# lixiaobai09/xgnn

Measured on AMD Instinct MI355X. Metric: sampled edges/s + feature-extract GB/s per epoch-step, higher is better.
Workload: dtype u32 ids / f32 rows (bit copy)

## Files before the change

### include/ggms.h

```cpp
#ifndef GGMS_H
#define GGMS_H

#include <stddef.h>
#include <stdint.h>

#ifdef __cplusplus
extern "C" {
#endif

typedef uint32_t ggms_id_t;
typedef void *ggms_stream_t;
typedef void *ggms_event_t;
#define GGMS_EMPTY_KEY 0xffffffffu

enum ggms_status {
  GGMS_OK = 0,
  GGMS_ERR_INVALID = -1,
  GGMS_ERR_HIP = -2,
  GGMS_ERR_NO_DEVICE = -3
};

enum ggms_dtype {
  GGMS_F32 = 0,
  GGMS_F64 = 1,
// ... 30 lines not shown
#define GGMS_DEBUG_GRID_CAP 3
#define GGMS_DEBUG_NUM_KNOBS 4
void ggms_debug_set_knob(int knob, long long value);
size_t ggms_dtype_bytes(int dtype);
size_t ggms_row_bytes(int dtype, size_t dim);

#define GGMS_MAX_PARTS 8
typedef struct {
  const ggms_id_t *indptr;
  const ggms_id_t *indices;
  const ggms_id_t *const *part_indptr;
  const ggms_id_t *const *part_indices;
  uint32_t num_part;
  uint32_t num_cache_node;
  uint32_t num_node;
  uint32_t _pad;
} ggms_graph_t;

#define GGMS_RNG_STATE_BYTES 24
int ggms_random_states_init(void *states, size_t num_states, uint64_t seed,
                            ggms_stream_t stream);
size_t ggms_random_states_count(int sample_type, const size_t *fanout,
                                size_t num_fanout, size_t batch_size,
                                size_t num_random_walk);

enum ggms_sample_type {
  GGMS_KHOP0 = 0,
  GGMS_KHOP1 = 1,
  GGMS_WEIGHTED_KHOP = 2,
  GGMS_RANDOM_WALK = 3,
  GGMS_WEIGHTED_KHOP_PREFIX = 4,
  GGMS_KHOP2 = 5,
// ... 439 lines not shown
```

### xgnn_amd/_lib.py

```python
import ctypes as C
import os

_HERE = os.path.dirname(os.path.abspath(__file__))
LIB_PATH = os.path.join(_HERE, "lib", "libggms_hip.so")
_LIB = None


class GgmsError(RuntimeError):
    pass


class Graph(C.Structure):
    _fields_ = [("indptr", C.c_void_p), ("indices", C.c_void_p),
                ("part_indptr", C.c_void_p), ("part_indices", C.c_void_p),
                ("num_part", C.c_uint32), ("num_cache_node", C.c_uint32),
                ("num_node", C.c_uint32), ("_pad", C.c_uint32)]


class SampleExtra(C.Structure):
    _fields_ = [("prob_table", C.c_void_p), ("alias_table", C.c_void_p), ("random_walk_length", C.c_size_t),
                ("random_walk_restart_prob", C.c_double), ("num_random_walk", C.c_size_t), ("data", C.c_void_p),
                ("rng_wait", C.c_void_p), ("rng_done", C.c_void_p), ("heavy_wait", C.c_void_p),
                ("seeds_distinct", C.c_uint32), ("labor_salt", C.c_uint32)]


class Temporal(C.Structure):
    _fields_ = [("edge_time", C.c_void_p), ("cut_table", C.c_void_p), ("stamp", C.c_uint32), ("pick", C.c_uint32)]


class Typed(C.Structure):
    _fields_ = [("edge_type", C.c_void_p), ("num_type", C.c_uint32), ("type_fanout", C.POINTER(C.c_uint32))]
# ... 56 lines not shown


_vp, _sz, _u64, _u32, _i = C.c_void_p, C.c_size_t, C.c_uint64, C.c_uint32, C.c_int
SYMBOLS = {
    "ggms_abi_version": (_i, []),
    "ggms_last_error": (C.c_char_p, []),
    "ggms_device_status": (_i, [C.POINTER(_u32), _i]),
    "ggms_debug_poison_next_scan": (None, []),
    "ggms_debug_set_scan_patience": (None, [C.c_uint32]),
    "ggms_debug_delay_next_scan": (None, [C.c_uint32]),
    "ggms_debug_set_scan_epoch": (C.c_uint32, [C.c_uint32]),
    "ggms_debug_set_knob": (None, [_i, C.c_longlong]),
    "ggms_fabric_probe": (_i, [_i, _vp, _sz, _sz, _u32, _vp, _vp]),
    "ggms_dtype_bytes": (_sz, [_i]),
    "ggms_row_bytes": (_sz, [_i, _sz]),
    "ggms_random_states_init": (_i, [_vp, _sz, _u64, _vp]),
    "ggms_random_states_count": (_sz, [_i, C.POINTER(_sz), _sz, _sz, _sz]),
    "ggms_sample_workspace_bytes": (_sz, [_i, _sz, _sz]),
    "ggms_sample_khop3": (_i, [C.POINTER(Graph), _vp, _sz, _sz, _vp, _vp, _vp, _vp, _sz, _vp, _sz, _vp]),
    "ggms_sample_khop0": (_i, [C.POINTER(Graph), _vp, _sz, _sz, _vp, _vp, _vp, _vp, _sz, _vp]),
    "ggms_sample_khop_labor": (_i, [C.POINTER(Graph), _vp, _sz, _sz, C.c_uint32, _vp, _vp, _vp, _vp, _sz, _vp]),
    "ggms_sample_khop_temporal": (_i, [C.POINTER(Graph), _vp, _vp, _vp, _sz, _sz, _i, C.c_uint32, _vp, _vp, _vp, _vp, _vp,
                                       _sz, _vp]),
    "ggms_sample_khop1": (_i, [C.POINTER(Graph), _vp, _sz, _sz, _vp, _vp, _vp, _vp, _sz, _vp, _sz, _vp]),
    "ggms_sample_khop2": (_i, [C.POINTER(Graph), _vp, _sz, _sz, _vp, _vp, _vp, _vp, _sz, _vp, _sz, _vp]),
    "ggms_sample_weighted_workspace_bytes": (_sz, [_sz, _sz]),
    "ggms_sample_weighted_khop": (_i, [C.POINTER(Graph), _vp, _vp, _vp, _sz, _sz, _vp, _vp, _vp, _vp, _sz, _vp, _sz,
                                       _vp]),
    "ggms_sample_weighted_khop_prefix": (_i, [C.POINTER(Graph), _vp, _vp, _sz, _sz, _vp, _vp, _vp, _vp, _sz, _vp, _sz,
                                              _vp]),
# ... 125 lines not shown
```

### xgnn_amd/csrc/engine/engine.cc

```cpp
#include "engine.h"
#include "team.h"
#include "../labor_hash.h"
#include "../row_formats.h"

#include <fcntl.h>
#include <pthread.h>
#include <sys/mman.h>
#include <signal.h>
#include <sys/stat.h>
#include <sys/wait.h>
#include <unistd.h>

#include <algorithm>
#include <atomic>
#include <chrono>
#include <condition_variable>
#include <cstdio>
#include <cstdlib>
#include <cstring>
#include <fstream>
#include <iostream>
#include <memory>
#include <mutex>
#include <random>
// ... 217 lines not shown
    const std::string v = kv["feat_store_dtype"];
    const auto name = kFeatDtypeNames.find(v);
    if (name == kFeatDtypeNames.end() || !ggms::quantiser_writes(name->second))
      fatal(__FILE__, __LINE__, "feat_store_dtype = " + v + ": unknown store type; the GPU quantiser writes F16, BF16, "
                                "F8E4M3, F8E5M2 or Q8ROW");
    cfg.feat_store_dtype = name->second;
    if (cfg.arch == kArch0)
      fatal(__FILE__, __LINE__, "arch0: feat_store_dtype needs a GPU: the table is encoded by a kernel, and the CPU engine "
                                "has no GPU; quantise the dataset offline (datagen.quantize_features)");
    if (cfg.arch == kArch5 || cfg.arch == kArch6)
      fatal(__FILE__, __LINE__, std::string(cfg.arch == kArch5 ? "arch5" : "arch6") + ": feat_store_dtype is not built: the "
                                "process that loads the dataset forks its workers and must not initialise the GPU before it "
                                "forks; quantise the dataset offline (datagen.quantize_features)");
    if (cfg.feat_store_dtype == GGMS_Q8ROW && cfg.feat_out_dtype < 0) fatal(__FILE__, __LINE__, kQ8RowNeedsOutDtype);
  }
  if (kv.count("task")) {
    const std::string v = kv["task"];
    if (v != "node_classification" && v != "link_prediction")
      fatal(__FILE__, __LINE__, "task = " + v + ": node_classification (the default) or link_prediction");
    cfg.link_prediction = v == "link_prediction";
  }
  if (cfg.link_prediction) {
    static const char *const arch_names[] = {"arch0", "arch1", "arch2", "arch3", "arch4", "arch5", "arch6", "arch7"};
    if (cfg.arch != kArch1)
      fatal(__FILE__, __LINE__, std::string(arch_names[cfg.arch]) + ": task = link_prediction is not built: edge seeds, "
                                "negative sampling and the pair ids run in arch1's sampling chain only");
    if (cfg.sample_type == GGMS_RANDOM_WALK)
      fatal(__FILE__, __LINE__, "task = link_prediction with _sample_type 3 (random_walk) is not built: the pair ids are "
                                "the k-hop batch's seed ids");
    if (kv.count("num_negative")) {
// ... 734 lines not shown
  void *d = nullptr;
  SAM_HIP(hipHostGetDevicePointer(&d, host, 0));
  return d;
}

void Engine::UploadGraph() {
  const uint32_t *indptr = (const uint32_t *)ds.indptr.ptr, *indices = (const uint32_t *)ds.indices.ptr;
  std::memset(&graph_, 0, sizeof(graph_));
  graph_.num_node = (uint32_t)ds.num_node;
  if (!cfg.use_dist_graph) {
    d_indptr_ = (uint32_t *)dev_upload(indptr, ds.indptr.bytes, stream_);
    d_indices_ = (uint32_t *)dev_upload(indices, ds.indices.bytes, stream_);
    graph_.indptr = d_indptr_;
    graph_.indices = d_indices_;
    SAM_HIP(hipStreamSynchronize(stream_));
    return;
  }
  const uint32_t P = (uint32_t)cfg.num_worker, p = (uint32_t)worker_id_;
  const uint32_t num_cache_edge = (uint32_t)(ds.num_edge * cfg.dist_graph_percentage);
  uint32_t num_cache_node = 0;
  while (num_cache_node < ds.num_node && indptr[num_cache_node] < num_cache_edge) ++num_cache_node;
  const size_t isz = num_cache_node / P + (p < num_cache_node % P ? 1 : 0) + 1;
  std::vector<uint32_t> pip(isz);
  size_t ecount = 0;
  for (uint32_t v = p; v < num_cache_node; v += P) ecount += indptr[v + 1] - indptr[v];
  std::vector<uint32_t> pix(std::max<size_t>(ecount, 1));
  uint32_t cnt = 0;
  for (uint32_t v = p; v < num_cache_node; v += P) {
    const uint32_t ne = indptr[v + 1] - indptr[v];
    pip[v / P] = cnt;
// ... 15 lines not shown
    for (uint32_t q = 0; q < P; ++q) {
      if (q == p) continue;
      part_indptr_[q] = OpenPeer(shared_->graph_indptr[q], q, shared_->indptr_words[q] * 4, "graph indptr shard");
      part_indices_[q] = OpenPeer(shared_->graph_indices[q], q, shared_->indices_words[q] * 4, "graph indices shard");
    }
    Barrier("graph shards opened");
  }
  part_indptr_[P] = dev_upload(ds.indptr.ptr, ds.indptr.bytes, stream_);
  SAM_HIP(hipStreamSynchronize(stream_));
  part_indices_[P] = (void *)map_host(ds.indices.ptr, ds.indices.bytes);
  SAM_CHECK(P <= GGMS_MAX_PARTS, "use_dist_graph: at most GGMS_MAX_PARTS topology shards");
  graph_.part_indptr = (const ggms_id_t *const *)part_indptr_.data();
  graph_.part_indices = (const ggms_id_t *const *)part_indices_.data();
  graph_.num_part = P;
  graph_.num_cache_node = num_cache_node;
}

void Engine::ComputeBounds() {
  const uint32_t L = (uint32_t)cfg.fanout.size();
  max_seeds_ = (size_t)(cfg.batch_size * 1.25) + 1;
  if (cfg.link_prediction) max_seeds_ = cfg.batch_size * (2 + cfg.num_negative);
  max_input_.resize(L);
  max_edges_.resize(L);
  SAM_GGMS(ggms_sample_batch_capacity(max_seeds_, cfg.fanout.data(), L, max_input_.data(), max_edges_.data(), &max_unique_));
  if (cfg.arch == kArch4)
    SAM_GGMS(ggms_sample_batch_prefetch_capacity(max_seeds_, cfg.fanout.data(), L, (const ggms_id_t *)ds.indptr.ptr,
                                                 ds.num_node, cfg.prefetch_max_edges, &max_prefetch_edges_, &max_unique_));
}

void Engine::SampleInit(int worker_id, const std::string &ctx) {
// ... 544 lines not shown
void Engine::Start() {
  if (Dedicated()) ExtractStart(0);
}

void Engine::Shutdown() {
  shutdown_ = true;
  bg_stop_ = true;
  pool_cv_.notify_all();
  if (bg_.joinable()) bg_.join();
  if (cfg.arch == kArch0) CpuShutdown();
  for (auto &P : pipes_)
    if (P.stream) (void)hipStreamSynchronize(P.stream);
  if (stream_) (void)hipStreamSynchronize(stream_);
  if (stream_extract_) (void)hipStreamSynchronize(stream_extract_);
  if (stream_extract2_) (void)hipStreamSynchronize(stream_extract2_);
}

Batch *Engine::AcquireSlot(bool background) {
  for (;;) {
    {
      std::lock_guard<std::mutex> lk(pool_mu_);
      for (auto &b : slots_)
        if (!b->in_use && b->refs.load() == 0) { b->in_use = true; return b.get(); }
    }
    if (bg_stop_) return nullptr;
    if (!background) return nullptr;
    std::this_thread::sleep_for(std::chrono::microseconds(20));
  }
}

// ... 505 lines not shown
```

### xgnn_amd/csrc/engine/engine.h

```cpp
#pragma once

#include <hip/hip_runtime.h>

#include <atomic>
#include <condition_variable>
#include <cstdint>
#include <deque>
#include <map>
#include <memory>
#include <mutex>
#include <string>
#include <thread>
#include <unordered_map>
#include <vector>

#include "../../../include/ggms.h"
#include "../../../include/samgraph.h"

namespace sam {

[[noreturn]] void fatal(const char *file, int line, const std::string &msg);
#define SAM_CHECK(cond, msg)                                   \
  do {                                                         \
    if (!(cond)) ::sam::fatal(__FILE__, __LINE__, std::string("Check failed: " #cond " ") + (msg)); \
// ... 35 lines not shown
  bool part_cache = false, gpu_extract = false;
  double replicate_percentage = 0.0;
  bool configured = false;
  bool has_seed = false;
  uint64_t seed = 0;
  uint64_t labor_seed = 0;
  bool direct_table = true;
  size_t lookahead = 2;
  size_t extract_streams = 2;
  size_t pipelines = 1;
  size_t presample_epoch = 0;
  bool dynamic_cache = false;
  size_t prefetch_max_edges = (size_t)1 << 26;
  int feat_out_dtype = -1;
  int feat_store_dtype = -1;
  bool link_prediction = false;
  uint32_t num_negative = 1;
  int negative_mode = GGMS_NEG_EXCLUDE;
  uint32_t exclude_seed_edges = 0;
  int feat_learnable = -1;
  float feat_lr = 0.0f, feat_eps = 1e-10f;
  bool edge_ids = false, edge_feat = false;
  int temporal_pick = GGMS_PICK_UNIFORM;
  bool Temporal() const { return sample_type == GGMS_KHOP_TEMPORAL; }
  std::vector<uint32_t> type_fanout;
  uint32_t num_edge_type = 0;
  bool Typed() const { return sample_type == GGMS_KHOP_TYPED; }
  bool SamplerEmitsEdgeIds() const { return Temporal() || Typed(); }
  bool induced = false;
  size_t induced_max_edges = 0;
// ... 151 lines not shown
  void *OpenPeer(const hipIpcMemHandle_t &handle, uint32_t peer, size_t bytes, const char *what);

 private:
  void LoadDataset();
  HostArray MapFile(const std::string &name, size_t bytes, bool to_shared_anon);
  void ShufflerInit();
  const uint32_t *SeedSet() const { return cfg.link_prediction ? ds.train_edges : (const uint32_t *)ds.train_set.ptr; }
  size_t SeedSetSize() const { return cfg.link_prediction ? ds.num_train_edge : ds.num_train; }
  uint64_t link_forced_ = 0;
  bool ShufflerNext(Batch *b, hipStream_t copy_stream);
  void Reshuffle();
  void DetectTopo();
  ggms_topology_t topo_{};
  bool topo_valid_ = false;
  void UploadGraph();
  void Presample();
  void QuantizeStore();
  void BuildCache();
  Batch *AcquireSlot(bool background);
  bool StagedHostTier() const { return cfg.arch == kArch6 && !cfg.gpu_extract && (cache_table_ != nullptr || !cfg.UseGPUCache()); }
  void StagedExtract(Batch *b, hipStream_t ss, hipStream_t xs);
  void HostGatherRows(char *rows, const uint32_t *ids, size_t first, size_t count);
  std::unique_ptr<class Team> host_team_;
  size_t staged_batches_ = 0;
  void SanityCheckBatch(const uint32_t *seeds, size_t n);
  std::vector<bool> sanity_seen_;
  uint32_t *node_access_dev_ = nullptr;
 public:
  void ReportNodeAccess();
 private:
// ... 25 lines not shown
  bool QueueWait(const uint64_t *word, uint64_t want, const char *what, bool stoppable);
  void PublishRanking();
  void WaitRankingReady();
  void Arch5TrainerInit(int worker_id, const std::string &ctx);
  void SendOne();
  bool Receive(Batch *b);
  void Unpack(Batch *b, hipStream_t xs);

  bool data_ready_ = false, sample_ready_ = false, train_ready_ = false, shutdown_ = false;
  int worker_id_ = 0, device_ = 0;
  int trainer_device_ = 0;
  hipStream_t stream_ = nullptr;
  hipStream_t stream_extract_ = nullptr;
  hipStream_t stream_extract2_ = nullptr;
  uint32_t *d_indptr_ = nullptr, *d_indices_ = nullptr;
  std::vector<void *> part_indptr_, part_indices_;
  ggms_graph_t graph_{};
  ggms_hashtable_t ht_{};
  ggms_sample_extra_t extra_{};
  void *d_prob_ = nullptr, *d_alias_ = nullptr;
  void *states_ = nullptr;
  size_t num_states_ = 0;
  void *ws_ = nullptr;
  size_t ws_bytes_ = 0;
  struct Pipe {
    hipStream_t stream = nullptr;
    ggms_hashtable_t ht{};
    void *ws = nullptr;
    hipEvent_t rng_done = nullptr;
    void *drop_ws = nullptr;
// ... 60 lines not shown
```

### xgnn_amd/csrc/ggms_device.h

```cpp
#pragma once
#include <cstdlib>

#include <hip/hip_runtime.h>
#include <stdint.h>

#include "../../include/ggms.h"

namespace ggms {

constexpr uint32_t kEmptyKey = GGMS_EMPTY_KEY;
constexpr int kWave = 64;
constexpr int kBlock = 256;
constexpr int kMaxGridBlocks = 2048;

void set_error(const char *fmt, ...);
#define GGMS_CHECK_ARG(cond)                                              \
  do {                                                                    \
    if (!(cond)) {                                                        \
      ::ggms::set_error("%s:%d: invalid argument: %s", __FILE__, __LINE__, #cond); \
      return GGMS_ERR_INVALID;                                            \
    }                                                                     \
  } while (0)
#define GGMS_HIP(call)                                                    \
  do {                                                                    \
// ... 56 lines not shown
  __device__ __forceinline__ T *pick(uint32_t k) const {
    T *r = p[0];
#pragma unroll 1
    for (uint32_t i = 1; i < N; ++i) r = (k == i) ? p[i] : r;
    return r;
  }
};

struct GraphView {
  const uint32_t *indptr;
  const uint32_t *indices;
  PtrSet<const uint32_t, kMaxParts + 1> pip, pix;
  Divisor part;
  uint32_t num_part;
  uint32_t num_cache_node;

  typedef uint32_t u32x2_a4 __attribute__((ext_vector_type(2), aligned(4)));
  static __device__ __forceinline__ void bounds(const uint32_t *ip, uint32_t v, uint32_t &b, uint32_t &e) {
    const u32x2_a4 be = *reinterpret_cast<const u32x2_a4 *>(ip + v);
    b = be.x;
    e = be.y;
  }
  __device__ __forceinline__ const uint32_t *neighbours(uint32_t v, uint32_t &len) const {
    if (num_part == 0) {
      uint32_t b, e;
      bounds(indptr, v, b, e);
      len = e - b;
      return indices + b;
    }
    uint32_t slot, real;
    part.divmod(v, real, slot);
    const bool cached = v < num_cache_node;
    slot = cached ? slot : kMaxParts;
    real = cached ? real : v;
    uint32_t b, e;
    bounds(pip.pick(slot), real, b, e);
    len = e - b;
    return pix.pick(slot) + b;
  }
};

bool host_readable_table(const void *table, const char *what);

inline bool view_of(const ggms_graph_t *g, GraphView &v) {
  v = GraphView{};
  v.indptr = g->indptr;
  v.indices = g->indices;
  v.num_part = g->num_part;
  v.num_cache_node = g->num_cache_node;
  v.part = divisor_of(g->num_part ? g->num_part : 1);
  if (g->num_part == 0) return true;
  if (g->num_part > kMaxParts || !g->part_indptr || !g->part_indices) {
    set_error("graph view: num_part %u (at most %u shards; part_indptr / part_indices are HOST arrays of num_part + 1 device pointers)",
              g->num_part, kMaxParts);
    return false;
  }
  if (!host_readable_table(g->part_indptr, "ggms_graph_t.part_indptr") ||
      !host_readable_table(g->part_indices, "ggms_graph_t.part_indices"))
    return false;
  for (uint32_t p = 0; p < g->num_part; ++p) {
    v.pip.p[p] = g->part_indptr[p];
    v.pix.p[p] = g->part_indices[p];
  }
  v.pip.p[kMaxParts] = g->part_indptr[g->num_part];
  v.pix.p[kMaxParts] = g->part_indices[g->num_part];
  return true;
// ... 134 lines not shown
```

### xgnn_amd/csrc/sample_khop.hip

```cpp
#include <algorithm>
#include <atomic>

#include "ggms_internal.h"

namespace ggms {

struct SeedCount {
  GraphView g;
  const uint32_t *input;
  uint32_t fanout;
  __device__ __forceinline__ uint32_t operator()(uint64_t i) const {
    uint32_t len;
    g.neighbours(input[i], len);
    return len < fanout ? len : fanout;
  }
};
struct StoreOffset {
  uint32_t *offset;
  __device__ __forceinline__ void operator()(uint64_t i, uint32_t, uint32_t excl) const { offset[i] = excl; }
};

template <int S>
__device__ __forceinline__ uint32_t row_shr(uint32_t v) {
  return (uint32_t)__builtin_amdgcn_update_dpp(0, (int)v, 0x110 + S, 0xf, 0xf, true);
}

struct Khop3TileHelp {
  static constexpr bool kCan = true;
  const GraphView &g;
  const uint32_t *input;
  uint64_t n;
  uint32_t fanout;
  __device__ __forceinline__ uint32_t operator()(uint64_t t) const {
    uint32_t acc = 0;
#pragma unroll
    for (uint32_t k = 0; k < 2; ++k) {
      const uint64_t i = 128 * t + 64 * k + (threadIdx.x & 63u);
      if (i < n) {
        uint32_t len;
        (void)g.neighbours(input[i], len);
        acc += len < fanout ? len : fanout;
      }
    }
    return wave_reduce_sum(acc);
  }
};

template <int GPW, bool INSERT, bool FIRST>
__global__ __launch_bounds__(128 * (4 / GPW), 6) void k_khop3_fused(GraphView g, const uint32_t *__restrict__ input,
                                                                 Count n_arg, uint32_t fanout, uint32_t fanout_magic,
                                                                 uint32_t *__restrict__ out_src,
                                                                 uint32_t *__restrict__ out_dst, SrcMode sm,
                                                                 uint32_t *__restrict__ states, uint32_t set_mask,
                                                                 uint32_t multi, FusedScan fs, DedupInsert di,
                                                                 FirstLayer fl) {
  constexpr uint32_t HASH_EMPTY = 0xffffffffu, NT = 128 * (4 / GPW), FLAG_A = 1, FLAG_P = 2;
  extern __shared__ uint32_t s_pos[];
  __shared__ uint32_t set_tab[8][128];
  __shared__ const uint32_t *s_ptr[128];
  __shared__ uint32_t s_len[128], s_rid[128], s_off[129];
  __shared__ uint64_t s_tile;
  __shared__ uint32_t s_prefix;
  const uint32_t lane = threadIdx.x & 63u;
  const bool active = GPW == 4 || lane < 16u * GPW;
  const uint64_t n = n_arg.get();
  if constexpr (FIRST) {
    if (blockIdx.x == 0) fl.pro.run(n, threadIdx.x, NT);
  }
  const uint32_t y = (threadIdx.x >> 6) * GPW + (lane >> 4), lig = lane & 15u;
  const uint32_t grp_shift = lane & ~15u;
  uint32_t *const tab = set_tab[active ? y : 0];
  const uint64_t num_tiles = (n + 127) / 128;
  const uint32_t my_s = y + 8u * lig;

  if (active)
    for (uint32_t s = lig; s <= set_mask; s += 16) tab[s] = HASH_EMPTY;
  bool dirty = false;

  const bool one_tile_each = gridDim.x >= num_tiles;
  for (uint32_t turn = 0;; ++turn) {
    if (one_tile_each) {
      if (turn != 0) break;
    } else {
      if (threadIdx.x == 0) s_tile = take_ticket(fs.tick);
      __syncthreads();
    }
    const uint64_t b = one_tile_each ? (uint64_t)blockIdx.x : s_tile;
    if (b >= num_tiles) break;
    uint32_t my_len = 0, my_magic = 0;
    unsigned long long seed_old = 0;
    if (active) {
      const uint64_t my_index = 128 * b + my_s;
      const uint32_t *ptr = nullptr;
      uint32_t rid = 0;
      if (my_index < n) {
        rid = input[my_index];
        if constexpr (FIRST) {
          fl.n2o[my_index] = rid;
          seed_old = atomicMin(di.w + rid, make_w1(di.version, 1u, (uint32_t)my_index));
        }
        ptr = g.neighbours(rid, my_len);
        if (my_len > fanout) my_magic = (uint32_t)(4294967296.0 / (double)my_len);
      }
      s_ptr[my_s] = ptr;
      s_len[my_s] = my_len;
      s_rid[my_s] = rid;
    }
    __syncthreads();
    if (threadIdx.x < kWave) {
      const uint32_t a = min(s_len[2 * lane], fanout), c = min(s_len[2 * lane + 1], fanout);
      const uint32_t incl = wave_inclusive_scan(a + c);
      s_off[2 * lane] = incl - (a + c);
      s_off[2 * lane + 1] = incl - c;
      if (lane == 63) {
        s_off[128] = incl;
        __hip_atomic_store(&fs.desc[b], scan_desc(fs.epoch, b == 0 ? FLAG_P : FLAG_A, incl), __ATOMIC_RELAXED,
// ... 100 lines not shown
        }
        if (lig == 0) st.store(states + 6 * stream);
      }
    }
    if constexpr (FIRST) {
      const uint64_t my_index = 128 * b + my_s;
      if (active && my_index < n) {
        const unsigned long long mine = make_w1(di.version, 1u, (uint32_t)my_index);
        const uint32_t idx = (uint32_t)seed_old;
        if (seed_old > mine && (seed_old >> 32) == (mine >> 32) && idx >= di.base) di.lost[idx - di.base] = di.tag;
      }
    }
    if (threadIdx.x < kWave) {
      uint32_t prefix = 0;
      if (b != 0) {
        prefix = scan_lookback(fs.desc, b, fs.epoch, fs.err, fs.patience, Khop3TileHelp{g, input, n, fanout});
        if (lane == 0)
          __hip_atomic_store(&fs.desc[b], scan_desc(fs.epoch, FLAG_P, prefix + s_off[128]), __ATOMIC_RELAXED,
                             __HIP_MEMORY_SCOPE_AGENT);
      }
      if (lane == 0) {
        s_prefix = prefix;
        if (b + 1 == num_tiles) *fs.num_out = (uint64_t)prefix + s_off[128];
      }
    }
    __syncthreads();
    const uint32_t prefix = s_prefix;
    const uint32_t slots = 128u * fanout;
    const auto slot_of = [&](uint32_t t, uint32_t &sd, uint32_t &e, uint32_t &pos) -> bool {
      sd = fanout == 1 ? t : __umulhi(t, fanout_magic);
      if (sd * fanout > t) --sd;
      const uint32_t j = t - sd * fanout;
      const uint32_t len = s_len[sd];
      if (j >= (len < fanout ? len : fanout)) return false;
      e = prefix + s_off[sd] + j;
      pos = len <= fanout ? j : s_pos[t];
      return true;
    };
    if (multi) {
      for (uint32_t t0 = threadIdx.x; t0 < slots; t0 += 4 * NT) {
        uint32_t sd[4], e[4], pos[4], nbr[4];
        bool ok[4];
#pragma unroll
        for (uint32_t u = 0; u < 4; ++u) {
          const uint32_t t = t0 + u * NT;
          ok[u] = t < slots && slot_of(t, sd[u], e[u], pos[u]);
          nbr[u] = ok[u] ? s_ptr[sd[u]][pos[u]] : 0u;
        }
        unsigned long long old[4];
#pragma unroll
        for (uint32_t u = 0; u < 4; ++u) {
          if (ok[u]) {
            out_src[e[u]] = sm.value(s_rid[sd[u]], 128 * b + sd[u]);
            out_dst[e[u]] = nbr[u];
            if (INSERT) old[u] = di.issue(nbr[u], e[u]);
          }
        }
        if (INSERT) {
#pragma unroll
          for (uint32_t u = 0; u < 4; ++u)
            if (ok[u]) di.finish(old[u], e[u]);
        }
      }
    } else {
      for (uint32_t t = threadIdx.x; t < slots; t += NT) {
        uint32_t sd, e, pos;
        if (!slot_of(t, sd, e, pos)) continue;
        const uint32_t nbr = s_ptr[sd][pos];
        out_src[e] = sm.value(s_rid[sd], 128 * b + sd);
        out_dst[e] = nbr;
        if (INSERT) di.enter(nbr, e);
      }
    }
    __syncthreads();
  }
  if (threadIdx.x == 0 && num_tiles == 0 && blockIdx.x == 0) *fs.num_out = 0;
}

struct Khop0Count {
  GraphView g;
  const uint32_t *input;
  uint32_t fanout;
  __device__ __forceinline__ U2 operator()(uint64_t i) const {
// ... 304 lines not shown
        out_dst[o[r] + j] = picked[r];
        indices[off[r] + sel[r]] = moved[r];
        indices[off[r] + tail[r]] = picked[r];
      }
    }
    st[3].store(states + 6 * sid);
  }
}

static int khop3_groups_per_wave(size_t blocks) { return blocks * 8 <= 2048 ? 1 : 2; }

size_t sample_ws_words(size_t num_input) {
  return num_input + tile_scan_words(num_input) + 16 + 2 * (num_input / 128 + 2) + kTicketWords + 16;
}

template <int GPW, bool INSERT, bool FIRST>
static int launch_khop3_fused(int grid, size_t lds, const SampleLayer &l, uint32_t set_mask, uint32_t multi,
                               FusedScan fs, DedupInsert di, FirstLayer fl) {
  const uint32_t fanout = (uint32_t)l.fanout;
  const uint32_t fanout_magic = (uint32_t)((0x100000000ull + fanout - 1) / fanout);
  if (lds > (48u << 10)) {
    static const int raised = raise_dynamic_lds(reinterpret_cast<const void *>(&k_khop3_fused<GPW, INSERT, FIRST>),
                                                128 * 127 * 4, "k_khop3_fused (fanout >= 96)");
    if (raised != GGMS_OK) return raised;
  }
  hipLaunchKernelGGL((k_khop3_fused<GPW, INSERT, FIRST>), dim3(grid), dim3(128 * (4 / GPW)), lds, l.s, l.g, l.input, l.n,
                     fanout, fanout_magic, l.out_src, l.out_dst, l.src, l.states, set_mask, multi, fs, di, fl);
  return GGMS_OK;
}

bool khop3_can_fuse_seeds(size_t num_seeds) { return (num_seeds + 127) / 128 <= grid_cap(); }

int sample_khop3_impl(const SampleLayer &l) {
  ScanArea *shared_scan = l.scan;
  const DedupInsert *insert = l.insert;
  const FirstLayer *first = l.first;
  const size_t tiles = (l.n_max + 127) / 128;
  if (first && (!insert || !shared_scan || !shared_scan->cleared || !khop3_can_fuse_seeds(l.n_max))) {
    set_error("sample_khop3: the fused first layer needs the batch's dedup insert, its scan area and one tile per workgroup");
    return GGMS_ERR_INVALID;
  }
  uint32_t *ctl = scan_align(shared_scan ? shared_scan->words : l.workspace);
  uint32_t *tick = shared_scan ? take_ticket_set(shared_scan) : ctl + 8 + 2 * (tiles + 1) + 2;
// ... 158 lines not shown
```

### xgnn_amd/ops.py

```python
import ctypes as C

import numpy as np

import torch

from . import _lib
from ._lib import Graph as _CGraph, HashTable as _CHashTable, check, lib
from ._lib import (COUNTS_SAMPLE_WORDS, COUNTS_WORDS, COUNT_DST, COUNT_EDGES, COUNT_EXPANSION, COUNT_INPUT, COUNT_SRC,
                   COUNT_STATUS)

EMPTY_KEY = 0xFFFFFFFF

DTYPE_CODE = {
    torch.float32: 0, torch.float64: 1, torch.float16: 2, torch.uint8: 3,
    torch.int32: 4, torch.int8: 5, torch.int64: 6, torch.int16: 2, torch.bfloat16: 7,
    torch.float8_e4m3fn: 16, torch.float8_e5m2: 17,
}

Q8ROW = 18


def _dtype_code(dtype):
    return dtype if isinstance(dtype, int) else DTYPE_CODE[dtype]

# ... 25 lines not shown
def _ptr(t):
    return C.c_void_p(t.data_ptr()) if t is not None else None


def _stream():
    return C.c_void_p(torch.cuda.current_stream().cuda_stream)


def _i32(t):
    assert t.dtype == torch.int32 and t.is_contiguous(), "ids must be contiguous int32 tensors"
    return t


class DeviceGraph:

    def __init__(self, indptr, indices, part_indptr=None, part_indices=None, num_cache_node=0):
        self.indptr, self.indices = indptr, indices
        self._keep = [indptr, indices]
        num_node = (indptr.numel() - 1) if indptr is not None else 0
        self.c = _CGraph()
        self.c.indptr = indptr.data_ptr() if indptr is not None else None
        self.c.indices = indices.data_ptr() if indices is not None else None
        self.c.num_node = num_node
        self.c.num_part = 0
        self.c.num_cache_node = 0
        if part_indptr is not None:
            self._pip = PartTable([t.data_ptr() for t in part_indptr])
            self._pix = PartTable([t.data_ptr() for t in part_indices])
            self._keep += list(part_indptr) + list(part_indices)
            self.c.part_indptr = self._pip.ptr().value
            self.c.part_indices = self._pix.ptr().value
            self.c.num_part = len(part_indptr) - 1
            self.c.num_cache_node = num_cache_node
            self.c.num_node = part_indptr[-1].numel() - 1


def random_states(num_states, seed, device="cuda"):
    st = torch.empty((num_states, 6), dtype=torch.int32, device=device)
    _require_gpu(st)
    check(lib().ggms_random_states_init(_ptr(st), num_states, seed, _stream()), "ggms_random_states_init")
    return st


def device_status(clear=False):
    st = C.c_uint32(0)
    check(lib().ggms_device_status(C.byref(st), 1 if clear else 0), "ggms_device_status")
    return st.value


# ... 191 lines not shown
def sample_weighted_khop_prefix(graph, prob_prefix_table, inp, fanout, states):
    return _sample("ggms_sample_weighted_khop_prefix", WEIGHTED_KHOP_PREFIX, graph, inp, fanout, states,
                   prob_prefix_table)


def sample_weighted_khop_hash_dedup(graph, prob_table, alias_table, inp, fanout, states):
    return _sample("ggms_sample_weighted_khop_hash_dedup", WEIGHTED_KHOP_HASH_DEDUP, graph, inp, fanout, states,
                   prob_table, alias_table)


def sample_khop1(graph, inp, fanout, states):
    return _sample("ggms_sample_khop1", KHOP1, graph, inp, fanout, states)


def sample_khop2(graph, inp, fanout, states):
    return _sample("ggms_sample_khop2", KHOP2, graph, inp, fanout, states)


def sample_weighted_khop(graph, prob_table, alias_table, inp, fanout, states):
    return _sample("ggms_sample_weighted_khop", WEIGHTED_KHOP, graph, inp, fanout, states, prob_table, alias_table)


def sample_random_walk(graph, inp, walk_length, restart_prob, num_walk, K, states):
    _require_gpu(inp)
    _i32(inp)
    n = inp.numel()
    dev = inp.device
    outs = [torch.empty(max(1, n * K), dtype=torch.int32, device=dev) for _ in range(3)]
    num_out = torch.zeros(1, dtype=torch.int64, device=dev)
    ws = _workspace(lib().ggms_sample_random_walk_workspace_bytes(n, walk_length, num_walk, K), dev)
# ... 441 lines not shown
            lib().ggms_ipc_release(C.c_void_p(p))
        self._imported = []

    def close(self):
        self.release_peers()
        if self.ptr:
            self.tensor = None
            lib().ggms_device_free(C.c_void_p(self.ptr))
            self.ptr = None


class _BatchBuffers:

    def _init_capacity(self, graph, fanouts, sample_type, max_seeds, prob_table, alias_table):
        self.graph, self.fanouts, self.sample_type = graph, [int(f) for f in fanouts], sample_type
        L = self.L = len(self.fanouts)
        self._f = (C.c_size_t * L)(*self.fanouts)
        self.max_seeds = max_seeds
        mi, me, mu = (C.c_size_t * L)(), (C.c_size_t * L)(), C.c_size_t(0)
        check(lib().ggms_sample_batch_capacity(max_seeds, self._f, L, mi, me, C.byref(mu)), "capacity")
        self.max_input, self.max_edges, self.max_unique = list(mi), list(me), mu.value
        self._keep = (prob_table, alias_table)
        self._extra = _lib.SampleExtra()
        self._extra.prob_table = prob_table.data_ptr() if prob_table is not None else None
        self._extra.alias_table = alias_table.data_ptr() if alias_table is not None else None

    def _init_states(self, stateless, seed, device, num_random_walk=0):
        nstates = lib().ggms_random_states_count(self.sample_type, self._f, self.L, self.max_seeds, num_random_walk)
        nstates = max(nstates, (max(self.max_input) + 127) // 128 * 8, (max(self.max_input) + 1023) // 1024 * 256)
        if self.sample_type == RANDOM_WALK:
# ... 297 lines not shown
```

Measured before the change: 5.132 billion.

## Add inline 64-byte per-node list heads for khop3 neighbour lookup

Builds a per-node 64-byte record holding the degree and either up to 15 neighbour ids inline or the list offset. The fused khop3 kernel reads one record instead of the indptr pair plus a separate indices gather, and copies short lists into LDS. The goal is fewer dependent global loads and fewer scattered accesses for low-degree nodes. In exchange it costs 64 bytes of device memory per node, extra LDS when fanout is below 15, a handle registry, and auto-enables only for khop3 when memory allows.

```diff
diff --git a/include/ggms.h b/include/ggms.h
--- a/include/ggms.h
+++ b/include/ggms.h
@@ -68,8 +68,17 @@
   uint32_t num_part;
   uint32_t num_cache_node;
   uint32_t num_node;
-  uint32_t _pad;
+  uint32_t heads_id;
 } ggms_graph_t;
+
+#define GGMS_LIST_HEAD_BYTES 64
+#define GGMS_LIST_HEAD_INLINE 15
+#define GGMS_LIST_HEADS_MAX 255
+size_t ggms_list_heads_bytes(size_t num_node);
+int ggms_list_heads_build(const ggms_graph_t *graph, void *heads, size_t bytes, ggms_stream_t stream);
+int ggms_list_heads_attach(ggms_graph_t *graph, const void *heads);
+int ggms_list_heads_detach(ggms_graph_t *graph);
+const void *ggms_list_heads_of(const ggms_graph_t *graph);
 
 #define GGMS_RNG_STATE_BYTES 24
 int ggms_random_states_init(void *states, size_t num_states, uint64_t seed,
diff --git a/xgnn_amd/_lib.py b/xgnn_amd/_lib.py
--- a/xgnn_amd/_lib.py
+++ b/xgnn_amd/_lib.py
@@ -14,7 +14,7 @@
     _fields_ = [("indptr", C.c_void_p), ("indices", C.c_void_p),
                 ("part_indptr", C.c_void_p), ("part_indices", C.c_void_p),
                 ("num_part", C.c_uint32), ("num_cache_node", C.c_uint32),
-                ("num_node", C.c_uint32), ("_pad", C.c_uint32)]
+                ("num_node", C.c_uint32), ("heads_id", C.c_uint32)]
 
 
 class SampleExtra(C.Structure):
@@ -101,6 +101,11 @@
     "ggms_fabric_probe": (_i, [_i, _vp, _sz, _sz, _u32, _vp, _vp]),
     "ggms_dtype_bytes": (_sz, [_i]),
     "ggms_row_bytes": (_sz, [_i, _sz]),
+    "ggms_list_heads_bytes": (_sz, [_sz]),
+    "ggms_list_heads_build": (_i, [C.POINTER(Graph), _vp, _sz, _vp]),
+    "ggms_list_heads_attach": (_i, [C.POINTER(Graph), _vp]),
+    "ggms_list_heads_detach": (_i, [C.POINTER(Graph)]),
+    "ggms_list_heads_of": (_vp, [C.POINTER(Graph)]),
     "ggms_random_states_init": (_i, [_vp, _sz, _u64, _vp]),
     "ggms_random_states_count": (_sz, [_i, C.POINTER(_sz), _sz, _sz, _sz]),
     "ggms_sample_workspace_bytes": (_sz, [_i, _sz, _sz]),
diff --git a/xgnn_amd/csrc/engine/engine.cc b/xgnn_amd/csrc/engine/engine.cc
--- a/xgnn_amd/csrc/engine/engine.cc
+++ b/xgnn_amd/csrc/engine/engine.cc
@@ -255,6 +255,14 @@
                                 "forks; quantise the dataset offline (datagen.quantize_features)");
     if (cfg.feat_store_dtype == GGMS_Q8ROW && cfg.feat_out_dtype < 0) fatal(__FILE__, __LINE__, kQ8RowNeedsOutDtype);
   }
+  if (kv.count("inline_heads")) {
+    const std::string v = kv["inline_heads"];
+    if (v != "auto" && v != "0" && v != "1") fatal(__FILE__, __LINE__, "inline_heads = " + v + ": auto (the default), 0 or 1");
+    cfg.inline_heads = v == "auto" ? -1 : (v == "1" ? 1 : 0);
+    if (cfg.inline_heads == 1 && (cfg.arch != kArch1 || cfg.use_dist_graph || cfg.sample_type == GGMS_KHOP2))
+      fatal(__FILE__, __LINE__, "inline_heads = 1: built for arch1 with the whole CSR on the GPU, and not beside khop2, "
+                                "which permutes the neighbour lists the table copies");
+  }
   if (kv.count("task")) {
     const std::string v = kv["task"];
     if (v != "node_classification" && v != "link_prediction")
@@ -1019,6 +1027,7 @@
     graph_.indptr = d_indptr_;
     graph_.indices = d_indices_;
     SAM_HIP(hipStreamSynchronize(stream_));
+    AttachListHeads();
     return;
   }
   const uint32_t P = (uint32_t)cfg.num_worker, p = (uint32_t)worker_id_;
@@ -1064,6 +1073,27 @@
   graph_.part_indices = (const ggms_id_t *const *)part_indices_.data();
   graph_.num_part = P;
   graph_.num_cache_node = num_cache_node;
+}
+
+void Engine::AttachListHeads() {
+  if (cfg.arch != kArch1 || cfg.inline_heads == 0 || ds.num_node == 0) return;
+  const size_t bytes = ggms_list_heads_bytes(ds.num_node);
+  if (cfg.inline_heads < 0) {
+    if (cfg.sample_type != GGMS_KHOP3) return;
+    size_t free_b = 0, total_b = 0;
+    SAM_HIP(hipMemGetInfo(&free_b, &total_b));
+    if (bytes > free_b / 4) {
+      std::fprintf(stderr, "[samgraph-amd] inline_heads = auto: not built (%zu bytes needed, %zu free: more than a quarter)\n",
+                   bytes, free_b);
+      return;
+    }
+  }
+  SAM_HIP(hipMalloc(&d_heads_, bytes));
+  SAM_GGMS(ggms_list_heads_build(&graph_, d_heads_, bytes, stream_));
+  SAM_HIP(hipStreamSynchronize(stream_));
+  SAM_GGMS(ggms_list_heads_attach(&graph_, d_heads_));
+  std::fprintf(stderr, "[samgraph-amd] inline_heads = %s: %zu bytes of list heads for %zu nodes attached\n",
+               cfg.inline_heads < 0 ? "auto" : "1", bytes, (size_t)ds.num_node);
 }
 
 void Engine::ComputeBounds() {
@@ -1638,6 +1668,7 @@
   if (stream_) (void)hipStreamSynchronize(stream_);
   if (stream_extract_) (void)hipStreamSynchronize(stream_extract_);
   if (stream_extract2_) (void)hipStreamSynchronize(stream_extract2_);
+  if (d_heads_) (void)ggms_list_heads_detach(&graph_);
 }
 
 Batch *Engine::AcquireSlot(bool background) {
diff --git a/xgnn_amd/csrc/engine/engine.h b/xgnn_amd/csrc/engine/engine.h
--- a/xgnn_amd/csrc/engine/engine.h
+++ b/xgnn_amd/csrc/engine/engine.h
@@ -73,6 +73,7 @@
   size_t prefetch_max_edges = (size_t)1 << 26;
   int feat_out_dtype = -1;
   int feat_store_dtype = -1;
+  int inline_heads = -1;
   bool link_prediction = false;
   uint32_t num_negative = 1;
   int negative_mode = GGMS_NEG_EXCLUDE;
@@ -254,6 +255,7 @@
   ggms_topology_t topo_{};
   bool topo_valid_ = false;
   void UploadGraph();
+  void AttachListHeads();
   void Presample();
   void QuantizeStore();
   void BuildCache();
@@ -309,6 +311,7 @@
   hipStream_t stream_extract_ = nullptr;
   hipStream_t stream_extract2_ = nullptr;
   uint32_t *d_indptr_ = nullptr, *d_indices_ = nullptr;
+  void *d_heads_ = nullptr;
   std::vector<void *> part_indptr_, part_indices_;
   ggms_graph_t graph_{};
   ggms_hashtable_t ht_{};
diff --git a/xgnn_amd/csrc/ggms_device.h b/xgnn_amd/csrc/ggms_device.h
--- a/xgnn_amd/csrc/ggms_device.h
+++ b/xgnn_amd/csrc/ggms_device.h
@@ -94,6 +94,7 @@
   Divisor part;
   uint32_t num_part;
   uint32_t num_cache_node;
+  const uint32_t *heads;
 
   typedef uint32_t u32x2_a4 __attribute__((ext_vector_type(2), aligned(4)));
   static __device__ __forceinline__ void bounds(const uint32_t *ip, uint32_t v, uint32_t &b, uint32_t &e) {
@@ -122,6 +123,9 @@
 
 bool host_readable_table(const void *table, const char *what);
 
+constexpr uint32_t kHeadWords = GGMS_LIST_HEAD_BYTES / 4, kHeadInline = GGMS_LIST_HEAD_INLINE;
+const uint32_t *list_heads_of(const ggms_graph_t *g);
+
 inline bool view_of(const ggms_graph_t *g, GraphView &v) {
   v = GraphView{};
   v.indptr = g->indptr;
@@ -129,7 +133,10 @@
   v.num_part = g->num_part;
   v.num_cache_node = g->num_cache_node;
   v.part = divisor_of(g->num_part ? g->num_part : 1);
-  if (g->num_part == 0) return true;
+  if (g->num_part == 0) {
+    if (g->heads_id != 0) v.heads = list_heads_of(g);
+    return true;
+  }
   if (g->num_part > kMaxParts || !g->part_indptr || !g->part_indices) {
     set_error("graph view: num_part %u (at most %u shards; part_indptr / part_indices are HOST arrays of num_part + 1 device pointers)",
               g->num_part, kMaxParts);
diff --git a/xgnn_amd/csrc/list_heads.hip b/xgnn_amd/csrc/list_heads.hip
--- /dev/null
+++ b/xgnn_amd/csrc/list_heads.hip
@@ -0,0 +1,123 @@
+#include <mutex>
+
+#include "ggms_internal.h"
+
+namespace ggms {
+
+namespace {
+
+__global__ __launch_bounds__(kBlock) void k_list_heads_build(const uint32_t *__restrict__ indptr,
+                                                             const uint32_t *__restrict__ indices, uint64_t num_node,
+                                                             uint4 *__restrict__ heads) {
+  const uint64_t quarters = 4 * num_node;
+  for (uint64_t t = (uint64_t)blockIdx.x * kBlock + threadIdx.x; t < quarters; t += (uint64_t)gridDim.x * kBlock) {
+    const uint64_t v = t >> 2;
+    const uint32_t w0 = 4u * ((uint32_t)t & 3u);
+    uint32_t b, e;
+    GraphView::bounds(indptr, (uint32_t)v, b, e);
+    const uint32_t deg = e - b;
+    uint32_t w[4];
+#pragma unroll
+    for (uint32_t k = 0; k < 4; ++k) {
+      const uint32_t i = w0 + k;
+      uint32_t x = 0;
+      if (i == 0) x = deg;
+      else if (deg <= kHeadInline) x = i <= deg ? indices[(uint64_t)b + i - 1] : 0u;
+      else if (i == 1) x = b;
+      w[k] = x;
+    }
+    heads[t] = make_uint4(w[0], w[1], w[2], w[3]);
+  }
+}
+
+struct HeadsEntry {
+  const void *heads;
+  const uint32_t *indptr, *indices;
+  uint32_t num_node;
+  bool live;
+};
+std::mutex g_heads_mutex;
+HeadsEntry g_heads[GGMS_LIST_HEADS_MAX + 1];
+
+void release_locked(uint32_t id) {
+  if (id >= 1 && id <= GGMS_LIST_HEADS_MAX) g_heads[id] = HeadsEntry{};
+}
+
+}
+
+const uint32_t *list_heads_of(const ggms_graph_t *g) {
+  const uint32_t id = g->heads_id;
+  if (id == 0 || id > GGMS_LIST_HEADS_MAX || g->num_part != 0) return nullptr;
+  std::lock_guard<std::mutex> lock(g_heads_mutex);
+  const HeadsEntry &h = g_heads[id];
+  if (!h.live || h.indptr != g->indptr || h.indices != g->indices || h.num_node != g->num_node) return nullptr;
+  return static_cast<const uint32_t *>(h.heads);
+}
+
+}
+
+using namespace ggms;
+
+extern "C" {
+
+size_t ggms_list_heads_bytes(size_t num_node) { return num_node * (size_t)GGMS_LIST_HEAD_BYTES; }
+
+int ggms_list_heads_build(const ggms_graph_t *graph, void *heads, size_t bytes, ggms_stream_t stream) {
+  GGMS_CHECK_ARG(graph);
+  if (graph->num_part != 0) {
+    set_error("ggms_list_heads_build: inline list heads are for unsharded graphs (num_part = %u)", graph->num_part);
+    return GGMS_ERR_INVALID;
+  }
+  if (graph->num_node == 0) return GGMS_OK;
+  GGMS_CHECK_ARG(graph->indptr && graph->indices && heads);
+  GGMS_CHECK_ARG(((uintptr_t)heads & (GGMS_LIST_HEAD_BYTES - 1)) == 0);
+  if (bytes < ggms_list_heads_bytes(graph->num_node)) {
+    set_error("ggms_list_heads_build: %zu bytes for %u nodes, %zu needed", bytes, graph->num_node,
+              ggms_list_heads_bytes(graph->num_node));
+    return GGMS_ERR_INVALID;
+  }
+  hipLaunchKernelGGL(k_list_heads_build, dim3(grid_for(4 * (size_t)graph->num_node, kBlock)), dim3(kBlock), 0,
+                     to_stream(stream), graph->indptr, graph->indices, (uint64_t)graph->num_node,
+                     static_cast<uint4 *>(heads));
+  GGMS_LAUNCH_CHECK();
+  return GGMS_OK;
+}
+
+int ggms_list_heads_attach(ggms_graph_t *graph, const void *heads) {
+  GGMS_CHECK_ARG(graph && heads);
+  GGMS_CHECK_ARG(((uintptr_t)heads & (GGMS_LIST_HEAD_BYTES - 1)) == 0);
+  if (graph->num_part != 0) {
+    set_error("ggms_list_heads_attach: inline list heads are for unsharded graphs (num_part = %u)", graph->num_part);
+    return GGMS_ERR_INVALID;
+  }
+  GGMS_CHECK_ARG(graph->indptr && graph->indices);
+  std::lock_guard<std::mutex> lock(g_heads_mutex);
+  const uint32_t old = graph->heads_id;
+  if (old >= 1 && old <= GGMS_LIST_HEADS_MAX && g_heads[old].live && g_heads[old].indptr == graph->indptr &&
+      g_heads[old].indices == graph->indices && g_heads[old].num_node == graph->num_node)
+    release_locked(old);
+  graph->heads_id = 0;
+  for (uint32_t id = 1; id <= GGMS_LIST_HEADS_MAX; ++id) {
+    if (g_heads[id].live) continue;
+    g_heads[id] = HeadsEntry{heads, graph->indptr, graph->indices, graph->num_node, true};
+    graph->heads_id = id;
+    return GGMS_OK;
+  }
+  set_error("ggms_list_heads_attach: all %d handles are in use", GGMS_LIST_HEADS_MAX);
+  return GGMS_ERR_INVALID;
+}
+
+const void *ggms_list_heads_of(const ggms_graph_t *graph) { return graph ? list_heads_of(graph) : nullptr; }
+
+int ggms_list_heads_detach(ggms_graph_t *graph) {
+  GGMS_CHECK_ARG(graph);
+  std::lock_guard<std::mutex> lock(g_heads_mutex);
+  const uint32_t id = graph->heads_id;
+  if (id >= 1 && id <= GGMS_LIST_HEADS_MAX && g_heads[id].live && g_heads[id].indptr == graph->indptr &&
+      g_heads[id].indices == graph->indices && g_heads[id].num_node == graph->num_node)
+    release_locked(id);
+  graph->heads_id = 0;
+  return GGMS_OK;
+}
+
+}
diff --git a/xgnn_amd/csrc/sample_khop.hip b/xgnn_amd/csrc/sample_khop.hip
--- a/xgnn_amd/csrc/sample_khop.hip
+++ b/xgnn_amd/csrc/sample_khop.hip
@@ -25,6 +25,7 @@
   return (uint32_t)__builtin_amdgcn_update_dpp(0, (int)v, 0x110 + S, 0xf, 0xf, true);
 }
 
+template <bool HEADS>
 struct Khop3TileHelp {
   static constexpr bool kCan = true;
   const GraphView &g;
@@ -38,7 +39,8 @@
       const uint64_t i = 128 * t + 64 * k + (threadIdx.x & 63u);
       if (i < n) {
         uint32_t len;
-        (void)g.neighbours(input[i], len);
+        if constexpr (HEADS) len = g.heads[(uint64_t)input[i] * kHeadWords];
+        else (void)g.neighbours(input[i], len);
         acc += len < fanout ? len : fanout;
       }
     }
@@ -46,7 +48,7 @@
   }
 };
 
-template <int GPW, bool INSERT, bool FIRST>
+template <int GPW, bool INSERT, bool FIRST, bool HEADS>
 __global__ __launch_bounds__(128 * (4 / GPW), 6) void k_khop3_fused(GraphView g, const uint32_t *__restrict__ input,
                                                                  Count n_arg, uint32_t fanout, uint32_t fanout_magic,
                                                                  uint32_t *__restrict__ out_src,
@@ -72,6 +74,8 @@
   uint32_t *const tab = set_tab[active ? y : 0];
   const uint64_t num_tiles = (n + 127) / 128;
   const uint32_t my_s = y + 8u * lig;
+  uint32_t *const s_nbr = fanout >= kHeadInline ? s_pos : s_pos + 128u * fanout;
+  const uint32_t nbr_stride = fanout >= kHeadInline ? fanout : kHeadInline;
 
   if (active)
     for (uint32_t s = lig; s <= set_mask; s += 16) tab[s] = HASH_EMPTY;
@@ -99,7 +103,22 @@
           fl.n2o[my_index] = rid;
           seed_old = atomicMin(di.w + rid, make_w1(di.version, 1u, (uint32_t)my_index));
         }
-        ptr = g.neighbours(rid, my_len);
+        if constexpr (HEADS) {
+          const uint4 *rec = reinterpret_cast<const uint4 *>(g.heads + (uint64_t)rid * kHeadWords);
+          const uint4 q0 = rec[0], q1 = rec[1], q2 = rec[2], q3 = rec[3];
+          my_len = q0.x;
+          if (my_len > kHeadInline) {
+            ptr = g.indices + q0.y;
+          } else if (my_len != 0) {
+            uint32_t *d = s_nbr + my_s * nbr_stride;
+            d[0] = q0.y; d[1] = q0.z; d[2] = q0.w;
+            d[3] = q1.x; d[4] = q1.y; d[5] = q1.z; d[6] = q1.w;
+            d[7] = q2.x; d[8] = q2.y; d[9] = q2.z; d[10] = q2.w;
+            d[11] = q3.x; d[12] = q3.y; d[13] = q3.z; d[14] = q3.w;
+          }
+        } else {
+          ptr = g.neighbours(rid, my_len);
+        }
         if (my_len > fanout) my_magic = (uint32_t)(4294967296.0 / (double)my_len);
       }
       s_ptr[my_s] = ptr;
@@ -230,7 +249,7 @@
     if (threadIdx.x < kWave) {
       uint32_t prefix = 0;
       if (b != 0) {
-        prefix = scan_lookback(fs.desc, b, fs.epoch, fs.err, fs.patience, Khop3TileHelp{g, input, n, fanout});
+        prefix = scan_lookback(fs.desc, b, fs.epoch, fs.err, fs.patience, Khop3TileHelp<HEADS>{g, input, n, fanout});
         if (lane == 0)
           __hip_atomic_store(&fs.desc[b], scan_desc(fs.epoch, FLAG_P, prefix + s_off[128]), __ATOMIC_RELAXED,
                              __HIP_MEMORY_SCOPE_AGENT);
@@ -243,7 +262,7 @@
     __syncthreads();
     const uint32_t prefix = s_prefix;
     const uint32_t slots = 128u * fanout;
-    const auto slot_of = [&](uint32_t t, uint32_t &sd, uint32_t &e, uint32_t &pos) -> bool {
+    const auto slot_of = [&](uint32_t t, uint32_t &sd, uint32_t &e, uint32_t &pos, bool &inl) -> bool {
       sd = fanout == 1 ? t : __umulhi(t, fanout_magic);
       if (sd * fanout > t) --sd;
       const uint32_t j = t - sd * fanout;
@@ -251,17 +270,24 @@
       if (j >= (len < fanout ? len : fanout)) return false;
       e = prefix + s_off[sd] + j;
       pos = len <= fanout ? j : s_pos[t];
+      inl = HEADS && len <= kHeadInline;
       return true;
+    };
+    const auto nbr_of = [&](uint32_t sd, uint32_t pos, bool inl) -> uint32_t {
+      if constexpr (HEADS) {
+        if (inl) return s_nbr[sd * nbr_stride + pos];
+      }
+      return s_ptr[sd][pos];
     };
     if (multi) {
       for (uint32_t t0 = threadIdx.x; t0 < slots; t0 += 4 * NT) {
         uint32_t sd[4], e[4], pos[4], nbr[4];
-        bool ok[4];
+        bool ok[4], inl[4];
 #pragma unroll
         for (uint32_t u = 0; u < 4; ++u) {
           const uint32_t t = t0 + u * NT;
-          ok[u] = t < slots && slot_of(t, sd[u], e[u], pos[u]);
-          nbr[u] = ok[u] ? s_ptr[sd[u]][pos[u]] : 0u;
+          ok[u] = t < slots && slot_of(t, sd[u], e[u], pos[u], inl[u]);
+          nbr[u] = ok[u] ? nbr_of(sd[u], pos[u], inl[u]) : 0u;
         }
         unsigned long long old[4];
 #pragma unroll
@@ -281,8 +307,9 @@
     } else {
       for (uint32_t t = threadIdx.x; t < slots; t += NT) {
         uint32_t sd, e, pos;
-        if (!slot_of(t, sd, e, pos)) continue;
-        const uint32_t nbr = s_ptr[sd][pos];
+        bool inl;
+        if (!slot_of(t, sd, e, pos, inl)) continue;
+        const uint32_t nbr = nbr_of(sd, pos, inl);
         out_src[e] = sm.value(s_rid[sd], 128 * b + sd);
         out_dst[e] = nbr;
         if (INSERT) di.enter(nbr, e);
@@ -617,19 +644,29 @@
   return num_input + tile_scan_words(num_input) + 16 + 2 * (num_input / 128 + 2) + kTicketWords + 16;
 }
 
+template <int GPW, bool INSERT, bool FIRST, bool HEADS>
+static int launch_khop3_fused_h(int grid, size_t lds, const SampleLayer &l, uint32_t set_mask, uint32_t multi,
+                                 FusedScan fs, DedupInsert di, FirstLayer fl) {
+  const uint32_t fanout = (uint32_t)l.fanout;
+  const uint32_t fanout_magic = (uint32_t)((0x100000000ull + fanout - 1) / fanout);
+  if (lds > (48u << 10)) {
+    static const int raised = raise_dynamic_lds(reinterpret_cast<const void *>(&k_khop3_fused<GPW, INSERT, FIRST, HEADS>),
+                                                128 * 127 * 4, "k_khop3_fused (fanout >= 96)");
+    if (raised != GGMS_OK) return raised;
+  }
+  hipLaunchKernelGGL((k_khop3_fused<GPW, INSERT, FIRST, HEADS>), dim3(grid), dim3(128 * (4 / GPW)), lds, l.s, l.g, l.input,
+                     l.n, fanout, fanout_magic, l.out_src, l.out_dst, l.src, l.states, set_mask, multi, fs, di, fl);
+  return GGMS_OK;
+}
+
 template <int GPW, bool INSERT, bool FIRST>
 static int launch_khop3_fused(int grid, size_t lds, const SampleLayer &l, uint32_t set_mask, uint32_t multi,
                                FusedScan fs, DedupInsert di, FirstLayer fl) {
-  const uint32_t fanout = (uint32_t)l.fanout;
-  const uint32_t fanout_magic = (uint32_t)((0x100000000ull + fanout - 1) / fanout);
-  if (lds > (48u << 10)) {
-    static const int raised = raise_dynamic_lds(reinterpret_cast<const void *>(&k_khop3_fused<GPW, INSERT, FIRST>),
-                                                128 * 127 * 4, "k_khop3_fused (fanout >= 96)");
-    if (raised != GGMS_OK) return raised;
-  }
-  hipLaunchKernelGGL((k_khop3_fused<GPW, INSERT, FIRST>), dim3(grid), dim3(128 * (4 / GPW)), lds, l.s, l.g, l.input, l.n,
-                     fanout, fanout_magic, l.out_src, l.out_dst, l.src, l.states, set_mask, multi, fs, di, fl);
-  return GGMS_OK;
+  if (l.g.heads) {
+    if (l.fanout < kHeadInline) lds += 128 * kHeadInline * sizeof(uint32_t);
+    return launch_khop3_fused_h<GPW, INSERT, FIRST, true>(grid, lds, l, set_mask, multi, fs, di, fl);
+  }
+  return launch_khop3_fused_h<GPW, INSERT, FIRST, false>(grid, lds, l, set_mask, multi, fs, di, fl);
 }
 
 bool khop3_can_fuse_seeds(size_t num_seeds) { return (num_seeds + 127) / 128 <= grid_cap(); }
diff --git a/xgnn_amd/ops.py b/xgnn_amd/ops.py
--- a/xgnn_amd/ops.py
+++ b/xgnn_amd/ops.py
@@ -63,8 +63,9 @@
 
 class DeviceGraph:
 
-    def __init__(self, indptr, indices, part_indptr=None, part_indices=None, num_cache_node=0):
+    def __init__(self, indptr, indices, part_indptr=None, part_indices=None, num_cache_node=0, inline_heads=None):
         self.indptr, self.indices = indptr, indices
+        self.heads = None
         self._keep = [indptr, indices]
         num_node = (indptr.numel() - 1) if indptr is not None else 0
         self.c = _CGraph()
@@ -82,6 +83,37 @@
             self.c.num_part = len(part_indptr) - 1
             self.c.num_cache_node = num_cache_node
             self.c.num_node = part_indptr[-1].numel() - 1
+        if inline_heads or inline_heads is None:
+            self._build_heads(required=bool(inline_heads))
+
+    def _build_heads(self, required):
+        on_gpu = (self.c.num_part == 0 and self.indptr is not None and self.indices is not None
+                  and getattr(self.indptr, "is_cuda", False) and getattr(self.indices, "is_cuda", False)
+                  and self.c.num_node > 0)
+        if not on_gpu:
+            if required:
+                raise _lib.GgmsError("inline_heads=True needs an unsharded CSR in device memory")
+            return
+        nbytes = lib().ggms_list_heads_bytes(self.c.num_node)
+        with torch.cuda.device(self.indptr.device):
+            if not required and 4 * nbytes > torch.cuda.mem_get_info()[0]:
+                return
+            heads = torch.empty(nbytes // 4, dtype=torch.int32, device=self.indptr.device)
+            check(lib().ggms_list_heads_build(C.byref(self.c), _ptr(heads), nbytes, _stream()), "ggms_list_heads_build")
+            torch.cuda.current_stream().synchronize()
+        check(lib().ggms_list_heads_attach(C.byref(self.c), _ptr(heads)), "ggms_list_heads_attach")
+        self.heads = heads
+
+    def detach_heads(self):
+        if self.heads is not None:
+            lib().ggms_list_heads_detach(C.byref(self.c))
+            self.heads = None
+
+    def __del__(self):
+        try:
+            self.detach_heads()
+        except Exception:
+            pass
 
 
 def random_states(num_states, seed, device="cuda"):
@@ -303,6 +335,7 @@
 
 
 def sample_khop2(graph, inp, fanout, states):
+    graph.detach_heads()
     return _sample("ggms_sample_khop2", KHOP2, graph, inp, fanout, states)
 
 
@@ -774,6 +807,8 @@
 
     def _init_capacity(self, graph, fanouts, sample_type, max_seeds, prob_table, alias_table):
         self.graph, self.fanouts, self.sample_type = graph, [int(f) for f in fanouts], sample_type
+        if sample_type == KHOP2:
+            graph.detach_heads()
         L = self.L = len(self.fanouts)
         self._f = (C.c_size_t * L)(*self.fanouts)
         self.max_seeds = max_seeds
```

Measured after the change: 5.365 billion, median of 6. +4.5%, better.
